# ruanhuabin/DataCompressionFloat

Hardware: AMD Instinct MI355X
Metric: compress + decompress GB/s (input floats), bit-exact round trip (higher is better)
Workload: dtype u8

## Files before the change

datacompressionfloat_amd/_lib.py:

```python
import ctypes
import os

_HERE = os.path.dirname(os.path.abspath(__file__))
LIB_PATH = os.environ.get("MRCZ_LIB_PATH") or os.path.join(_HERE, "lib", "libmrcz_hip.so")


class MrczLibraryMissing(ImportError):
    pass


class MrczBoxGeom(ctypes.Structure):
    _fields_ = [("data_word0", ctypes.c_uint64), ("nx", ctypes.c_uint32), ("ny", ctypes.c_uint32), ("nz", ctypes.c_uint32),
                ("bx", ctypes.c_uint32), ("by", ctypes.c_uint32), ("bz", ctypes.c_uint32), ("fill_bits", ctypes.c_uint32)]


class MrczBinGeom(ctypes.Structure):
    _fields_ = [("data_word0", ctypes.c_uint64), ("nx", ctypes.c_uint32), ("ny", ctypes.c_uint32), ("nz", ctypes.c_uint32),
                ("fx", ctypes.c_uint32), ("fy", ctypes.c_uint32), ("fz", ctypes.c_uint32)]


class MrczCompare(ctypes.Structure):
    _fields_ = [(k, ctypes.c_uint64) for k in ("n", "n_header_diff", "n_diff", "n_finite", "n_special_diff", "n_over_abs", "n_over_rel",
                                               "first_over", "max_err_index", "max_rel_index")] + \
               [(k, ctypes.c_double) for k in ("max_err", "max_rel", "sum_err", "sum_abs_err", "sum_err2", "orig_min", "orig_max",
# ... 39 lines not shown
    lib.mrcz_record_size.restype = i32
    lib.mrcz_record_size.argtypes = [vp, u32, ctypes.POINTER(u64)]
    lib.mrcz_records_index.restype = i32
    lib.mrcz_records_index.argtypes = [vp, u64, u64, u32, ctypes.POINTER(u64)]
    lib.mrcz_uncompress_range.restype = i32
    lib.mrcz_uncompress_range.argtypes = [vp, vp, u64, u64, u32, u64, u64, u64, vp, i32, ctypes.POINTER(u64)]
    geom = ctypes.POINTER(MrczBoxGeom)
    lib.mrcz_box_origins.restype = i32
    lib.mrcz_box_origins.argtypes = [geom, vp, u32, vp]
    lib.mrcz_boxes_chunks.restype = i32
    lib.mrcz_boxes_chunks.argtypes = [geom, vp, u32, u64, u32, vp]
    lib.mrcz_uncompress_boxes.restype = i32
    lib.mrcz_uncompress_boxes.argtypes = [vp, vp, u64, u64, u32, u64, u64, geom, vp, u32, vp, i32, ctypes.POINTER(u64)]
    bgeom = ctypes.POINTER(MrczBinGeom)
    lib.mrcz_bin_chunks.restype = i32
    lib.mrcz_bin_chunks.argtypes = [bgeom, u64, u32, ctypes.POINTER(u64), ctypes.POINTER(u64)]
    lib.mrcz_uncompress_binned.restype = i32
    lib.mrcz_uncompress_binned.argtypes = [vp, vp, u64, u64, u32, u64, u64, bgeom, vp, i32, ctypes.POINTER(u64)]
    lib.mrcz_binned_finish.restype = i32
    lib.mrcz_binned_finish.argtypes = [vp, bgeom, vp, vp]
    lib.mrcz_uncompress_compare.restype = i32
    lib.mrcz_uncompress_compare.argtypes = [vp, vp, u64, u64, u32, u64, u64, vp, ctypes.c_double, ctypes.c_double, i32, vp]
    lib.mrcz_compare_finish.restype = i32
    lib.mrcz_compare_finish.argtypes = [vp, vp, u64, u64, ctypes.POINTER(MrczCompare)]
    lib.mrcz_crc32_combine.restype = u32
    lib.mrcz_crc32_combine.argtypes = [u32, u32, u64]
    lib.mrcz_uncompress_digest.restype = i32
    lib.mrcz_uncompress_digest.argtypes = [vp, vp, u64, u64, u32, u64, u64, i32, vp]
    for f in (lib.mrcz_digest_words, lib.mrcz_digest_words_async):
        f.restype = i32
        f.argtypes = [vp, vp, u64, u64, u32, i32, i32, ctypes.c_float, vp]
    lib.mrcz_digest_finish.restype = i32
    lib.mrcz_digest_finish.argtypes = [vp, vp, u64, u64, ctypes.POINTER(MrczDigest)]
    lib.mrcz_record_top_span.restype = i32
    lib.mrcz_record_top_span.argtypes = [vp, u32, i32, ctypes.POINTER(u64), ctypes.POINTER(u64)]
    lib.mrcz_uncompress_top.restype = i32
    lib.mrcz_uncompress_top.argtypes = [vp, vp, u64, u64, u32, u64, u64, i32, i32, vp, ctypes.POINTER(u64)]
    lib.mrcz_generate_kat_words.restype = i32
    lib.mrcz_generate_kat_words.argtypes = [vp, vp, u64, u64]
    lib.mrcz_set_ztypes.restype = i32
    lib.mrcz_set_ztypes.argtypes = [vp, ctypes.c_char_p]
    lib.mrcz_erase_bits.restype = i32
    lib.mrcz_erase_bits.argtypes = [vp, vp, u64, u64, i32]
    lib.mrcz_erase_abs.restype = i32
    lib.mrcz_erase_abs.argtypes = [vp, vp, u64, u64, ctypes.c_float]
    lib.mrcz_set_timing.restype = i32
    lib.mrcz_set_timing.argtypes = [vp, i32]
    lib.mrcz_last_timings.restype = i32
    lib.mrcz_last_timings.argtypes = [vp, ctypes.POINTER(ctypes.c_char_p), ctypes.POINTER(ctypes.c_float), i32]
    lib.mrcz_debug_fallbacks.restype = ctypes.c_int64
    lib.mrcz_debug_fallbacks.argtypes = [vp]
    lib.mrcz_debug_chain_fallbacks.restype = ctypes.c_int64
    lib.mrcz_debug_chain_fallbacks.argtypes = [vp]
    return lib


EXPORTS = [
    "mrcz_create", "mrcz_destroy", "mrcz_last_error", "mrcz_stream", "mrcz_records_bound",
    "mrcz_compress_chunks", "mrcz_uncompress_chunks", "mrcz_erase_bits", "mrcz_set_timing",
    "mrcz_last_timings", "mrcz_debug_blocks", "mrcz_debug_fallbacks", "mrcz_debug_chain_fallbacks", "mrcz_debug_inflate_phases", "mrcz_debug_candidates", "mrcz_device_count", "mrcz_dev_malloc", "mrcz_dev_free",
    "mrcz_host_malloc", "mrcz_host_free", "mrcz_copy_h2d", "mrcz_copy_d2h",
    "mrcz_event_create", "mrcz_event_destroy", "mrcz_event_record", "mrcz_stream_wait_event", "mrcz_event_sync",
    "mrcz_copy_h2d_async", "mrcz_copy_d2h_async", "mrcz_compress_chunks_async", "mrcz_uncompress_chunks_async",
    "mrcz_set_ztypes", "mrcz_generate_kat_words", "mrcz_err_hist", "mrcz_err_collect", "mrcz_compress_chunks_int8", "mrcz_uncompress_chunks_int8", "mrcz_compress_chunks_int8_async", "mrcz_uncompress_chunks_int8_async",
    "mrcz_record_size", "mrcz_records_index", "mrcz_uncompress_range", "mrcz_uncompress_range_async",
    "mrcz_box_origins", "mrcz_boxes_chunks", "mrcz_uncompress_boxes",
    "mrcz_bin_chunks", "mrcz_uncompress_binned", "mrcz_binned_finish",
    "mrcz_compress_chunks_abs", "mrcz_compress_chunks_abs_async", "mrcz_erase_abs",
    "mrcz_uncompress_compare", "mrcz_compare_finish",
    "mrcz_crc32_combine", "mrcz_uncompress_digest", "mrcz_digest_words", "mrcz_digest_words_async", "mrcz_digest_finish",
    "mrcz_record_top_span", "mrcz_uncompress_top", "mrcz_uncompress_top_async",
]
```

datacompressionfloat_amd/csrc/mrcz_api.hip:

```cpp
#include "mrcz_compress.hip"
#include "mrcz_huffman.hip"
#include "mrcz_inflate.hip"
#include "mrcz_inflate_par.hip"
#include "mrcz_tools.hip"

#include "../../include/mrcz_hip.h"

#include <math.h>
#include <stdio.h>
#include <stdlib.h>
#include <string.h>
#include <time.h>

using namespace mrcz;

#define MAX_TIMERS 32

constexpr int MAX_LANES = 2;
constexpr uint32_t SPLIT_PCT = 55;
constexpr uint32_t HIST_FEW = 8;
constexpr uint32_t BLK_WGS_PER_CU = 3;
static uint32_t validate_grid(uint32_t ns) { return ns * 192u < 4096u ? 4096u : ns * 192u > 32768u ? 32768u : ns * 192u; }

namespace mrcz { struct CmpPart; }
// ... 278 lines not shown
    if (!(eps > 0.0f) || !isfinite(eps)) return fail(ctx, MRCZ_EINVAL, "absolute error bound must be finite and > 0", hipSuccess);
    uint32_t bits;
    memcpy(&bits, &eps, 4);
    const int32_t e = (int32_t)(bits >> 23);
    ae->q = e ? e - 127 : -150 + (32 - __builtin_clz(bits));
    ae->E = bits;
    return MRCZ_OK;
}

static int ensure_planes(mrcz_ctx *ctx)
{
    if (ctx->planes) return MRCZ_OK;
    hipError_t e = hipMalloc((void **)&ctx->planes, (size_t)4 * ctx->row_chunks * CHK);
    if (e != hipSuccess) { ctx->planes = NULL; return fail(ctx, MRCZ_ENOMEM, "plane workspace", e); }
    return MRCZ_OK;
}

static int compress_lane(mrcz_ctx *ctx, hipStream_t lstream, int phase, int slot, uint32_t s0, const uint32_t *bin, uint64_t bfl,
                         uint32_t nb, uint32_t mask, uint32_t fstart, uint8_t *out, Xform xf, AbsErr ae)
{
    const uint32_t ns = 4u * nb;
    TileSum *tsum = ctx->tsum + (size_t)s0 * TPS;
    TileInfo *tinfo = ctx->tinfo + (size_t)s0 * TPS;
    StreamInfo *sinfo = ctx->sinfo + s0;
    uint32_t *blkstart = ctx->blkstart + (size_t)s0 * (MAXBLK + 1);
    uint32_t *slideq = ctx->slideq + (size_t)s0 * MAXSLIDE;
    uint16_t *pairhist = ctx->pairhist + (size_t)s0 * MAXPAIR * HROW;
    uint16_t *blkfreq = ctx->blkfreq + (size_t)s0 * MAXBLK * HROW;
    uint32_t *blkcode = ctx->blkcode + (size_t)s0 * MAXBLK * HROW;
    uint32_t *blkhdr = ctx->blkhdr + (size_t)s0 * MAXBLK * HDRWORDS;
    BlkMeta *meta = ctx->meta + (size_t)s0 * MAXBLK;
    BlkLay *lay = ctx->lay + (size_t)s0 * MAXBLK;
    uint32_t *pairbits = ctx->pairbits + (size_t)s0 * MAXPAIR;
    uint32_t *pairoff = ctx->pairoff + (size_t)s0 * MAXPAIR;
    uint32_t *blkbase = ctx->blkbase + s0 + (uint32_t)slot;
    uint8_t *planes = ctx->planes + (size_t)s0 * CHK;
    if (phase == 0) {
        if (xf == Xform::Quant) LAUNCH("k_tile_summary", k_tile_summary<Xform::Quant>, dim3(SPS, nb), dim3(256), bin, bfl, mask, fstart, tsum, planes);
        else if (xf == Xform::AbsErr) LAUNCH("k_tile_summary", k_tile_summary<Xform::AbsErr>, dim3(SPS, nb), dim3(256), bin, bfl, ae, fstart, tsum, planes);
        else LAUNCH("k_tile_summary", k_tile_summary<Xform::Mask>, dim3(SPS, nb), dim3(256), bin, bfl, mask, fstart, tsum, planes);
        LAUNCH("k_stream_scan", k_stream_scan, dim3(ns), dim3(256), tsum, bfl, tinfo, sinfo, blkstart);
        if (nb <= 12u) LAUNCH("k_histogram", k_histogram<4>, dim3(SPS, nb, 4), dim3(256), planes, bfl, tinfo, pairhist, blkstart, slideq, HIST_FEW);
        else LAUNCH("k_histogram", k_histogram<1>, dim3(SPS, nb, 4), dim3(64), planes, bfl, tinfo, pairhist, blkstart, slideq, HIST_FEW);
        LAUNCH("k_block_reduce", k_block_reduce, dim3(MAXBLK, ns), dim3(64), tinfo, sinfo, pairhist, blkfreq);
        LAUNCH("k_block_index", k_block_index, dim3(1), dim3(256), sinfo, ns, blkbase);
        HIPCHK(hipEventRecord(ctx->ev_stream[slot], lstream), "event");
        unsigned long long *hdbg = ctx->phase_profile == 3 ? ctx->dbgphase : (unsigned long long *)NULL;
        LAUNCH("k_huffman", k_huffman, dim3((ns * MAXBLK + HUFF_TREES - 1) / HUFF_TREES), dim3(HUFF_TREES), sinfo, ns, blkbase, blkfreq, blkcode, blkhdr, meta, hdbg);
        LAUNCH("k_huffman_hdr", k_huffman_hdr, dim3(ns * MAXBLK), dim3(64), sinfo, ns, blkbase, blkcode, blkhdr, meta);
        LAUNCH("k_stream_layout", k_stream_layout, dim3(ns), dim3(64), sinfo, meta, blkstart, slideq, lay);
        LAUNCH("k_pair_bits", k_pair_bits, dim3(SPS, ns), dim3(64), sinfo, lay, pairhist, blkcode, tinfo, pairbits);
        LAUNCH("k_pair_offsets", k_pair_offsets, dim3(ns), dim3(64), sinfo, lay, tinfo, pairbits, pairoff);
    } else if (phase == 1) {
        LAUNCH("k_container", k_container, dim3(1), dim3(256), sinfo, nb, out, ctx->result, 0, slot);
    } else {
        LAUNCH("k_zero_records", k_zero_records, dim3(2048), dim3(256), out, ctx->result, slot);
        LAUNCH("k_container", k_container, dim3(1), dim3(256), sinfo, nb, out, ctx->result, 1, slot);
        LAUNCH("k_emit", k_emit, dim3(SPS, nb, 4), dim3(64), planes, bfl, tinfo, sinfo, lay, blkstart, blkcode, pairoff, out);
        LAUNCH("k_emit_headers", k_emit_headers, dim3(MAXBLK + 1, ns), dim3(64), sinfo, lay, meta, blkhdr, blkstart, out);
    }
    return MRCZ_OK;
}

static int compress_enqueue(mrcz_ctx_t *ctx, const void *d_in, uint64_t nfloats, uint64_t first_chunk, int bits, void *d_out, uint64_t out_cap,
                            uint64_t *h_res, Xform xf, AbsErr ae = AbsErr{})
{
    if (!ctx || !d_in || !d_out || !h_res) return MRCZ_EINVAL;
    if (bits < 0 || bits > 32) return fail(ctx, MRCZ_EINVAL, "bits outside 0..32 (reference table has 33 entries, workers.c:29-37)", hipSuccess);
    if (((uintptr_t)d_in & 15u) || ((uintptr_t)d_out & 3u)) return fail(ctx, MRCZ_EINVAL, "d_in must be 16-byte and d_out 4-byte aligned", hipSuccess);
    ctx->ntimers = 0;
    if (nfloats == 0) return fail(ctx, MRCZ_EINVAL, "nothing to compress", hipSuccess);
    const uint64_t bound = mrcz_records_bound(nfloats);
    if (out_cap < bound) return fail(ctx, MRCZ_ECAP, "output capacity below mrcz_records_bound()", hipSuccess);
    HIPCHK(hipSetDevice(ctx->device), "hipSetDevice");
    const uint32_t mask = mask_of(bits);
    const uint64_t nchunks = (nfloats + CHK - 1) / CHK;
    const uint32_t *in = (const uint32_t *)d_in;
    uint8_t *out = (uint8_t *)d_out;
    if (int rc = ensure_planes(ctx)) return rc;
    HIPCHK(hipMemsetAsync(ctx->result, 0, 16 * sizeof(uint64_t), ctx->stream), "memset result");
    HIPCHK(hipEventRecord(ctx->ev_start, ctx->stream), "event");
    for (uint32_t l = 1; l < ctx->lanes; l++) HIPCHK(hipStreamWaitEvent(ctx->lane_stream[l], ctx->ev_start, 0), "wait");
    bool cont_pending = false;
    uint32_t prev_lanes = 0, prev_lc0[MAX_LANES + 1] = {0};
    int stream_pending = -1;
    for (uint64_t c0 = 0; c0 < nchunks; c0 += ctx->max_chunks) {
        const uint32_t nb = (uint32_t)((nchunks - c0) < ctx->max_chunks ? (nchunks - c0) : ctx->max_chunks);
        const uint32_t nlanes = (ctx->timing || nb < 8u) ? 1u : ctx->lanes;
        const uint64_t bfl = (nfloats - c0 * CHK) < (uint64_t)nb * CHK ? (nfloats - c0 * CHK) : (uint64_t)nb * CHK;
        ctx->last_streams = 4u * nb;
        ctx->last_nlanes = nlanes;
        uint32_t lc0[MAX_LANES + 1] = {0u, nb};
        if (nlanes == 2u) {
            lc0[1] = (uint32_t)(((uint64_t)nb * SPLIT_PCT + 50u) / 100u);
            if (lc0[1] < 1u) lc0[1] = 1u;
            if (lc0[1] > nb - 1u) lc0[1] = nb - 1u;
            lc0[2] = nb;
        }
        bool same_rows = prev_lanes == nlanes;
        for (uint32_t l = 0; same_rows && l < nlanes; l++) same_rows = prev_lc0[l] == lc0[l];
        if (prev_lanes && !same_rows) {
            for (uint32_t l = 0; l < prev_lanes; l++) HIPCHK(hipEventRecord(ctx->ev_done[l], ctx->lane_stream[l]), "event");
            for (uint32_t l = 0; l < nlanes; l++)
                for (uint32_t k = 0; k < prev_lanes; k++)
                    if (k != l) HIPCHK(hipStreamWaitEvent(ctx->lane_stream[l], ctx->ev_done[k], 0), "wait");
        }
        prev_lanes = nlanes;
        for (uint32_t l = 0; l <= nlanes; l++) prev_lc0[l] = lc0[l];
        for (int phase = 0; phase < 3; phase++) {
            for (uint32_t l = 0; l < nlanes; l++) {
                const uint32_t cb = lc0[l], nbl = lc0[l + 1] - lc0[l];
// ... 502 lines not shown
    return MRCZ_OK;
}

extern "C" int mrcz_err_collect(mrcz_ctx_t *ctx, const void *d_orig, const void *d_dec, uint64_t n, uint64_t base_index, uint32_t threshold_bits,
                                void *d_points, uint64_t cap_points, uint64_t count_in, uint64_t *count_out)
{
    if (!ctx || !d_orig || !d_dec || !d_points || !count_out) return MRCZ_EINVAL;
    HIPCHK(hipSetDevice(ctx->device), "hipSetDevice");
    ctx->ntimers = 0;
    hipStream_t lstream = ctx->stream;
    if (!ctx->errhist) {
        hipError_t e = hipMalloc((void **)&ctx->errhist, 2049 * sizeof(unsigned long long));
        if (e != hipSuccess) { ctx->errhist = NULL; return fail(ctx, MRCZ_ENOMEM, "error histogram", e); }
    }
    unsigned long long *cnt = ctx->errhist + 2048;
    unsigned long long start = count_in;
    HIPCHK(hipMemcpyAsync(cnt, &start, sizeof(start), hipMemcpyHostToDevice, ctx->stream), "copy count");
    if (n) LAUNCH("k_err_collect", k_err_collect, dim3(2048), dim3(256), (const uint32_t *)d_orig, (const uint32_t *)d_dec, n, base_index, threshold_bits,
                  (ErrPoint *)d_points, cnt, cap_points);
    unsigned long long got = 0;
    HIPCHK(hipMemcpyAsync(&got, cnt, sizeof(got), hipMemcpyDeviceToHost, ctx->stream), "copy count");
    HIPCHK(hipStreamSynchronize(ctx->stream), "stream sync (collect)");
    *count_out = got;
    return MRCZ_OK;
}

extern "C" int mrcz_debug_inflate_phases(mrcz_ctx_t *ctx, int enable, uint32_t stream, uint64_t out[20])
{
    if (!ctx) return MRCZ_EINVAL;
    ctx->phase_profile = enable;
    if (enable == 3 && !out && hipMemset(ctx->dbgphase, 0, 40 * sizeof(unsigned long long)) != hipSuccess) return MRCZ_EHIP;
    if (out) {
        if (stream >= 8u * ctx->max_chunks) return MRCZ_EINVAL;
        if (hipMemcpy(out, ctx->dbgphase + (size_t)stream * 20, 20 * sizeof(uint64_t), hipMemcpyDeviceToHost) != hipSuccess) return MRCZ_EHIP;
    }
    return MRCZ_OK;
}

extern "C" int mrcz_debug_candidates(mrcz_ctx_t *ctx, uint64_t out[2])
{
    if (!ctx || !out) return MRCZ_EINVAL;
    uint32_t raw[RAW_SEGS];
    if (hipMemcpy(raw, ctx->njobs + 4, sizeof(raw), hipMemcpyDeviceToHost) != hipSuccess) return MRCZ_EHIP;
    out[0] = 0;
    for (uint32_t g = 0; g < RAW_SEGS; g++) out[0] += raw[g];
    out[1] = 0;
    uint32_t nc[512];
    const uint32_t ns = 4u * (ctx->max_chunks < 128u ? ctx->max_chunks : 128u);
    if (hipMemcpy(nc, ctx->ncand, ns * sizeof(uint32_t), hipMemcpyDeviceToHost) != hipSuccess) return MRCZ_EHIP;
    for (uint32_t s = 0; s < ns; s++) out[1] += nc[s];
    return MRCZ_OK;
}

extern "C" int64_t mrcz_debug_fallbacks(const mrcz_ctx_t *ctx) { return ctx ? (int64_t)ctx->last_fallbacks : -1; }
extern "C" int64_t mrcz_debug_chain_fallbacks(mrcz_ctx_t *ctx) { return ctx ? (int64_t)ctx->last_chain_fallbacks : -1; }

extern "C" int mrcz_debug_blocks(mrcz_ctx_t *ctx, uint32_t stream, mrcz_block_info_t *blocks, uint32_t max_blocks)
{
    if (!ctx || stream >= ctx->last_streams) return MRCZ_EINVAL;
    {
        uint32_t l = 0;
        while (l + 1 < ctx->last_nlanes && (stream >> 2) >= ctx->last_lc0[l + 1]) l++;
        stream = ctx->last_row0[l] + (stream - 4u * ctx->last_lc0[l]);
    }
    StreamInfo si;
    if (hipMemcpy(&si, ctx->sinfo + stream, sizeof(si), hipMemcpyDeviceToHost) != hipSuccess) return MRCZ_EHIP;
    uint32_t nb = si.nblk;
    if (nb > (uint32_t)MAXBLK) return MRCZ_EFORMAT;
    BlkLay *lay = (BlkLay *)malloc(sizeof(BlkLay) * (nb + 1));
    BlkMeta *meta = (BlkMeta *)malloc(sizeof(BlkMeta) * (nb + 1));
    uint32_t *bs = (uint32_t *)malloc(sizeof(uint32_t) * (nb + 2));
    (void)hipMemcpy(lay, ctx->lay + (size_t)stream * MAXBLK, sizeof(BlkLay) * nb, hipMemcpyDeviceToHost);
    (void)hipMemcpy(meta, ctx->meta + (size_t)stream * MAXBLK, sizeof(BlkMeta) * nb, hipMemcpyDeviceToHost);
    (void)hipMemcpy(bs, ctx->blkstart + (size_t)stream * (MAXBLK + 1), sizeof(uint32_t) * (nb + 1), hipMemcpyDeviceToHost);
    for (uint32_t b = 0; b < nb && b < max_blocks; b++) {
        blocks[b].start = bs[b];
        blocks[b].end = bs[b + 1];
        blocks[b].btype = lay[b].btype;
        blocks[b].opt_len = meta[b].opt_len;
        blocks[b].static_len = meta[b].static_len;
        blocks[b].bitpos = lay[b].bitpos;
    }
    free(lay); free(meta); free(bs);
    return (int)nb;
}
```

datacompressionfloat_amd/csrc/mrcz_compress.hip:

```cpp
#include "mrcz_tile.h"

namespace mrcz {

template <Xform X>
__global__ __launch_bounds__(256) void k_tile_summary(const uint32_t *__restrict__ in, uint64_t nfloats,
                                                      typename XformArg<X>::type mask, uint32_t first_chunk_is_file_start,
                                                      TileSum *__restrict__ tsum, uint8_t *__restrict__ planes)
{
    __shared__ __attribute__((aligned(16))) uint8_t lds[4 * PLANE_LDS];
    const uint32_t g = blockIdx.x, c = blockIdx.y;
    const uint64_t cbase = (uint64_t)c * CHK;
    const uint32_t n = (uint32_t)((nfloats - cbase) < CHK ? (nfloats - cbase) : CHK);
    if ((uint64_t)g * SEG >= n) return;
    const uint32_t *cin = in + cbase;
    const uint32_t unmasked = (c == 0 && first_chunk_is_file_start) ? 256u : 0u;
    const int lane = lane_id(), w = threadIdx.x >> 6;
    const uint32_t s = 4u * c + (uint32_t)w;

    for (int ti = 0; ti < TILES_PER_SEG; ti++) {
        const uint32_t t0 = g * SEG + ti * TILE;
        if (t0 >= n) break;
        const int len = (int)((n - t0) < (uint32_t)TILE ? (n - t0) : (uint32_t)TILE);
        stage_tile<X>(cin, t0, (uint32_t)len, mask, unmasked, lds);
        __syncthreads();
// ... 566 lines not shown
    }
}

__global__ __launch_bounds__(64) void k_pair_offsets(const StreamInfo *__restrict__ sinfo, const BlkLay *__restrict__ lay,
                                                     const TileInfo *__restrict__ tinfo, const uint32_t *__restrict__ pairbits,
                                                     uint32_t *__restrict__ pairoff)
{
    __shared__ uint32_t s_val[MAXPAIR];
    __shared__ uint8_t s_head[MAXPAIR];
    const uint32_t s = blockIdx.x;
    const StreamInfo si = sinfo[s];
    const int lane = lane_id();
    const TileInfo *ti = tinfo + (size_t)s * TPS;
    const uint32_t npair = si.nseg ? si.nseg + si.nsym / BLK_SYMS : 0u;
    for (uint32_t g = lane; g < si.nseg; g += 64) {
        const uint32_t bs = ti[g * TILES_PER_SEG].P / BLK_SYMS;
        const uint32_t be = ((g + 1 < si.nseg) ? ti[(g + 1) * TILES_PER_SEG].P : si.nsym) / BLK_SYMS;
        for (uint32_t b = bs; b <= be; b++) {
            const uint32_t i = g + b;
            if (i >= (uint32_t)MAXPAIR) break;
            const bool head = b > bs || g == 0u;
            s_head[i] = head ? 1 : 0;
            s_val[i] = head ? (b < si.nblk ? lay[(size_t)s * MAXBLK + b].databit : 0u) : pairbits[(size_t)s * MAXPAIR + i - 1u];
        }
    }
    __builtin_amdgcn_wave_barrier();
    constexpr int R = (MAXPAIR + 63) / 64;
    const uint32_t per = (npair + 63u) / 64u;
    const uint32_t i0 = (uint32_t)lane * per;
    uint32_t sum = 0, flag = 0;
#pragma unroll
    for (int r = 0; r < R; r++) {
        const uint32_t i = i0 + (uint32_t)r;
        if ((uint32_t)r >= per || i >= npair) continue;
        if (s_head[i]) { sum = s_val[i]; flag = 1; } else sum += s_val[i];
    }
    uint32_t isum = sum, iflag = flag;
    for (int d = 1; d < 64; d <<= 1) {
        const uint32_t os = (uint32_t)__shfl_up((int)isum, d), of = (uint32_t)__shfl_up((int)iflag, d);
        if (lane >= d) { if (!iflag) isum += os; iflag |= of; }
    }
    uint32_t run = (uint32_t)__shfl_up((int)isum, 1);
    if (lane == 0) run = 0;
    uint32_t *po = pairoff + (size_t)s * MAXPAIR;
#pragma unroll
    for (int r = 0; r < R; r++) {
        const uint32_t i = i0 + (uint32_t)r;
        if ((uint32_t)r >= per || i >= npair) continue;
        run = s_head[i] ? s_val[i] : run + s_val[i];
        po[i] = run;
    }
}

__global__ __launch_bounds__(256) void k_zero_records(uint8_t *__restrict__ out, const uint64_t *__restrict__ result, int slot)
{
    uint8_t *b = out + result[8 + slot], *e = out + result[12 + slot];
    uint8_t *ba = reinterpret_cast<uint8_t *>(((uintptr_t)b + 15u) & ~(uintptr_t)15u);
    uint8_t *ea = reinterpret_cast<uint8_t *>((uintptr_t)e & ~(uintptr_t)15u);
    if (ba > e) ba = e;
    if (ea < ba) ea = ba;
    if (blockIdx.x == 0 && threadIdx.x < 16u && b + threadIdx.x < ba) b[threadIdx.x] = 0;
    if (blockIdx.x == 1 && threadIdx.x < 16u && ea + threadIdx.x < e) ea[threadIdx.x] = 0;
    uint4 *p = reinterpret_cast<uint4 *>(ba);
    const uint64_t n = (uint64_t)(ea - ba) >> 4;
    const uint4 z = make_uint4(0, 0, 0, 0);
    for (uint64_t i = (uint64_t)blockIdx.x * 256u + threadIdx.x; i < n; i += (uint64_t)gridDim.x * 256u) p[i] = z;
}

__global__ __launch_bounds__(256) void k_container(StreamInfo *__restrict__ sinfo, uint32_t nchunks, uint8_t *__restrict__ out,
                                                   uint64_t *__restrict__ result ,
                                                   int write_headers, int slot)
{
    __shared__ SegPair wsum[4];
    const uint32_t c = threadIdx.x;
    uint32_t len[4] = {0, 0, 0, 0}, raw[4] = {0, 0, 0, 0};
    SegPair v;
    v.sum = 0;
    v.brk = 0;
    if (c < nchunks) {
        for (int j = 0; j < 4; j++) {
            len[j] = sinfo[4 * c + j].paylen;
            raw[j] = sinfo[4 * c + j].raw;
        }
        v.sum = 16u + len[0] + len[1] + len[2] + len[3];
    }
    const uint64_t base = write_headers ? result[8 + slot] : result[0];
    const SegPair pre = block_excl_scan(v, wsum);
    if (c < nchunks) {
        const uint64_t off = base + pre.sum;
        uint64_t p = off + 16;
        for (int j = 0; j < 4; j++) {
            if (write_headers) {
                uint8_t *h = out + off + 4u * j;
                h[0] = (uint8_t)(len[j] & 0xff);
                h[1] = (uint8_t)((len[j] >> 8) & 0xff);
                h[2] = (uint8_t)((len[j] >> 16) & 0xff);
                h[3] = (uint8_t)(((len[j] >> 24) & 0x7f) | (raw[j] << 7));
            } else {
                sinfo[4 * c + j].payoff = p;
                atomicAdd((unsigned long long *)&result[1 + j], (unsigned long long)len[j] + 4ull);
            }
            p += len[j];
        }
    }
    __syncthreads();
    if (!write_headers && c + 1 == nchunks) {
        result[8 + slot] = base;
        result[12 + slot] = base + pre.sum + v.sum;
        result[0] = base + pre.sum + v.sum;
    }
}

constexpr int STAGE_WORDS = 1280;

__device__ __forceinline__ void global_or_bits(uint32_t *out32, uint64_t pos, uint32_t val, int nbits)
{
    if (nbits <= 0) return;
    const uint64_t wi = pos >> 5;
    const int sh = (int)(pos & 31u);
    const uint64_t v = (uint64_t)(nbits >= 32 ? val : (val & ((1u << nbits) - 1u))) << sh;
    if ((uint32_t)v) atomicOr(&out32[wi], (uint32_t)v);
    if ((uint32_t)(v >> 32)) atomicOr(&out32[wi + 1], (uint32_t)(v >> 32));
}

struct LanePacker {
    uint32_t *stage;
    uint64_t acc;
    int nacc;
    uint32_t word;
    int covered;
};
__device__ __forceinline__ void packer_init(LanePacker &p, uint32_t *stage, uint32_t bitpos)
{
    p.stage = stage;
    p.word = bitpos >> 5;
    p.covered = (int)(bitpos & 31u);
    p.acc = 0;
    p.nacc = 0;
}
__device__ __forceinline__ void packer_put(LanePacker &p, uint32_t val, int nbits)
{
    p.acc |= (uint64_t)val << (p.covered + p.nacc);
    p.nacc += nbits;
    if (p.covered + p.nacc >= 32) {
        const uint32_t wv = (uint32_t)p.acc;
        if (p.covered == 0) p.stage[p.word] = wv;
        else atomicOr(&p.stage[p.word], wv);
        p.acc >>= 32;
        p.nacc -= 32 - p.covered;
        p.covered = 0;
        p.word++;
    }
}
__device__ __forceinline__ void packer_finish(LanePacker &p)
{
    if (p.nacc > 0) atomicOr(&p.stage[p.word], (uint32_t)p.acc);
}

constexpr int EMIT_WAVES = 5;
#define OPAQUE4(x, q) asm volatile("" : "+v"((x)[4 * (q)]), "+v"((x)[4 * (q) + 1]), "+v"((x)[4 * (q) + 2]), "+v"((x)[4 * (q) + 3]))

__device__ __forceinline__ uint32_t quarter_byte(const uint32_t wv[4], int j)
// ... 8 lines not shown
    if (__ballot(Lg != 0xffffu) == 0ull) {
#pragma unroll
        for (int j = 0; j < 16; j++) bits += lut[(wv[j >> 2] >> (8 * (j & 3))) & 0xffu] >> 16;
    } else {
#pragma unroll
        for (int j = 0; j < 16; j++) {
            const uint32_t e = lut[(wv[j >> 2] >> (8 * (j & 3))) & 0xffu];
            bits += ((Lg >> j) & 1u) ? (e >> 16) : 0u;
        }
    }
    return bits;
}

__device__ __forceinline__ void quarter_emit(LanePacker &pk, const uint32_t *lut, const uint32_t wv[4], uint32_t Sg, uint32_t Mg,
                                             int q, const LaneTile &lt, uint32_t dbits)
{
    if (__ballot(Mg != 0u || Sg != 0xffffu) == 0ull) {
#pragma unroll
        for (int j = 0; j < 16; j += 2) {
            const uint32_t e0 = lut[(wv[j >> 2] >> (8 * (j & 3))) & 0xffu];
            const uint32_t e1 = lut[(wv[(j + 1) >> 2] >> (8 * ((j + 1) & 3))) & 0xffu];
            const uint32_t n0 = e0 >> 16;
            packer_put(pk, (e0 & 0xffffu) | ((e1 & 0xffffu) << n0), (int)(n0 + (e1 >> 16)));
        }
        return;
    }
    uint32_t rem = Sg;
    while (__ballot(rem != 0u)) {
        if (rem) {
            const int j = __builtin_ctz(rem);
            rem &= rem - 1u;
            uint32_t val;
            int nb;
            if ((Mg >> j) & 1u) {
                int xb, xv;
                const int code = len_code(match_len_at(lt.E, lt.a, lt.nextS, 16 * q + j), &xb, &xv);
                const uint32_t e = lut[257 + code];
                const int cl = (int)(e >> 16);
                val = (e & 0xffffu) | ((uint32_t)xv << cl);
                nb = cl + xb + (int)dbits;
            } else {
                const uint32_t e = lut[quarter_byte(wv, j)];
                val = e & 0xffffu;
                nb = (int)(e >> 16);
            }
            packer_put(pk, val, nb);
        }
    }
}

__global__ __launch_bounds__(64) __attribute__((amdgpu_waves_per_eu(EMIT_WAVES))) void k_emit(const uint8_t *__restrict__ planes, uint64_t nfloats, const TileInfo *__restrict__ tinfo,
                                              const StreamInfo *__restrict__ sinfo, const BlkLay *__restrict__ lay,
                                              const uint32_t *__restrict__ blkstart, const uint32_t *__restrict__ blkcode,
                                              const uint32_t *__restrict__ pairoff, uint8_t *__restrict__ out)
{
    __shared__ __attribute__((aligned(16))) uint32_t stage[STAGE_WORDS];
    __shared__ uint32_t lut[HROW];
    const uint32_t g = blockIdx.x, c = blockIdx.y;
    const uint64_t cbase = (uint64_t)c * CHK;
    const uint32_t n = (uint32_t)((nfloats - cbase) < CHK ? (nfloats - cbase) : CHK);
    if ((uint64_t)g * SEG >= n) return;
    const int lane = lane_id(), w = plane_of_slot(blockIdx.z);
    const uint32_t s = 4u * c + (uint32_t)w;
    const uint8_t *pl = planes + (size_t)s * CHK;
    const StreamInfo si = sinfo[s];
    uint32_t *out32 = reinterpret_cast<uint32_t *>(out);
    const uint64_t paybit = si.payoff * 8ull;
    const uint32_t *bstart = blkstart + (size_t)s * (MAXBLK + 1);
    const BlkLay *blay = lay + (size_t)s * MAXBLK;

    uint32_t curBlk = 0xffffffffu;
    uint32_t cur = 0;
    int mode = -1;
    uint32_t blkEnd = 0;
    uint32_t dbits = 0;

    for (int ti = 0; ti < TILES_PER_SEG; ti++) {
        const uint32_t t0 = g * SEG + ti * TILE;
        if (t0 >= n) break;
        const int len = (int)((n - t0) < (uint32_t)TILE ? (n - t0) : (uint32_t)TILE);
        uint32_t x[16];
        load_plane_row(pl, t0, len, lane, x);
        if (si.raw) {
            uint8_t *dst = out + si.payoff + t0 + 64u * (uint32_t)lane;
            const int mine = len - 64 * lane;
            if (mine >= 64) {
#pragma unroll
                for (int k = 0; k < 4; k++) {
                    const uint4 v = make_uint4(x[4 * k], x[4 * k + 1], x[4 * k + 2], x[4 * k + 3]);
                    __builtin_memcpy(dst + 16 * k, &v, 16);
                }
            } else {
                for (int i = 0; i < mine; i++) dst[i] = pl[t0 + 64u * (uint32_t)lane + (uint32_t)i];
            }
            continue;
        }
        const TileInfo tinf = tinfo[(size_t)s * TPS + (t0 / TILE)];
        const LaneTile lt = analyse_lane(x, lane, len, tinf.B, tinf.F);
        const LaneCls cls = classify_lane(lt.E, lt.a, lt.prevS, lt.nextS);
        if (curBlk == 0xffffffffu) {
            curBlk = tinf.P / BLK_SYMS;
            if (bstart[curBlk] > t0) curBlk--;
            mode = -1;
        }

        int pos0 = 0;
        int cap = len;
        for (int part = 0; part < 16 && pos0 < len; part++) {
            if (mode < 0 || t0 + (uint32_t)pos0 >= blkEnd) {
                if (mode >= 0) curBlk++;
                const BlkLay L = blay[curBlk];
                mode = (int)L.btype;
                blkEnd = bstart[curBlk + 1];
                if (mode == 0) cur = L.databit + 8u * (t0 + (uint32_t)pos0 - bstart[curBlk]);
                else {
                    __builtin_amdgcn_wave_barrier();
                    if (mode == 2) {
                        const uint32_t *code = blkcode + ((size_t)s * MAXBLK + curBlk) * HROW;
                        for (int i = lane; i < 286; i += 64) lut[i] = code[i];
                        dbits = 1;
                    } else {
                        for (int i = lane; i < 286; i += 64) {
                            int l;
                            const uint32_t cd = static_lcode(i, &l);
                            lut[i] = cd | ((uint32_t)l << 16);
                        }
                        dbits = 5;
                    }
                    cur = pairoff[(size_t)s * MAXPAIR + (g + curBlk)];
                    __builtin_amdgcn_wave_barrier();
                }
            }
            int pos1 = cap;
            if (blkEnd < t0 + (uint32_t)pos1) pos1 = (int)(blkEnd - t0);

            if (mode == 0) {
                const uint32_t nbytes = (uint32_t)(pos1 - pos0);
                const uint64_t dg = si.payoff + (cur >> 3);
                const uint32_t mis = (uint32_t)(dg & 3u);
                const uint64_t w0 = dg >> 2;
                const uint32_t nwords = (mis + nbytes + 3u) >> 2;
                const uint8_t *src = pl + t0 + (uint32_t)pos0;
                for (uint32_t k = lane; k < nwords; k += 64) {
                    uint32_t v = 0;
                    bool full = true;
#pragma unroll
                    for (int j = 0; j < 4; j++) {
                        const int rel = (int)(4u * k + (uint32_t)j) - (int)mis;
                        if (rel >= 0 && rel < (int)nbytes) v |= (uint32_t)src[rel] << (8 * j);
                        else full = false;
                    }
                    if (full) out32[w0 + k] = v;
                    else if (v) atomicOr(&out32[w0 + k], v);
                }
                cur += 8u * nbytes;
                pos0 = pos1; cap = len;
                continue;
            }
            const int lo = pos0 - lt.a, hi = pos1 - lt.a;
            const uint64_t mlo = lo <= 0 ? ~0ull : (lo >= 64 ? 0ull : (~0ull << lo));
            const uint64_t mhi = hi >= 64 ? ~0ull : (hi <= 0 ? 0ull : ((1ull << hi) - 1ull));
            const uint64_t pm = mlo & mhi & lt.V;
            const uint64_t S = cls.S & pm, M = cls.M & pm;

            if (__ballot(S != 0ull) == 0ull) { pos0 = pos1; cap = len; continue; }
            uint32_t lbits = 0;
            {
                const uint64_t L = S & ~M;
#pragma unroll
                for (int q = 0; q < 4; q++) {
                    const uint32_t Lg = (uint32_t)(L >> (16 * q)) & 0xffffu;
                    if (__ballot(Lg != 0u) == 0ull) continue;
                    OPAQUE4(x, q);
                    lbits += quarter_literal_bits(lut, &x[4 * q], Lg);
                }
                uint64_t m = M;
                while (m) {
                    const int i = ctz64(m); m &= m - 1;
                    int xb, xv;
                    const int code = len_code(match_len_at(lt.E, lt.a, lt.nextS, i), &xb, &xv);
                    lbits += (lut[257 + code] >> 16) + (uint32_t)xb + dbits;
                }
            }
            uint32_t tot;
            const uint32_t lofs = wave_excl_sum(lbits, &tot);
            if (tot) {
                const uint64_t gbit = paybit + cur;
                const uint32_t lead = (uint32_t)(gbit & 31u);
                const uint32_t nwords = (lead + tot + 31u) >> 5;
                if (nwords > (uint32_t)STAGE_WORDS) {
                    cap = pos0 + ((((pos1 - pos0) >> 1) + 63) & ~63);
                    continue;
                }
                for (uint32_t i = lane; i < nwords; i += 64) stage[i] = 0;
                __builtin_amdgcn_wave_barrier();
                LanePacker pk;
                packer_init(pk, stage, lead + lofs);
#pragma unroll
                for (int q = 0; q < 4; q++) {
                    const uint32_t Sg = (uint32_t)(S >> (16 * q)) & 0xffffu, Mg = (uint32_t)(M >> (16 * q)) & 0xffffu;
                    if (__ballot(Sg != 0u) == 0ull) continue;
                    OPAQUE4(x, q);
                    quarter_emit(pk, lut, &x[4 * q], Sg, Mg, q, lt, dbits);
                }
                packer_finish(pk);
                __builtin_amdgcn_wave_barrier();
                const uint64_t w0 = gbit >> 5;
                for (uint32_t i = lane; i < nwords; i += 64) {
                    const uint32_t v = stage[i];
                    if (i == 0 || i == nwords - 1) { if (v) atomicOr(&out32[w0 + i], v); }
                    else out32[w0 + i] = v;
                }
                __builtin_amdgcn_wave_barrier();
                cur += tot;
            }
            pos0 = pos1; cap = len;
        }
    }
}

__global__ __launch_bounds__(64) void k_emit_headers(const StreamInfo *__restrict__ sinfo, const BlkLay *__restrict__ lay,
                                                     const BlkMeta *__restrict__ meta, const uint32_t *__restrict__ blkhdr,
                                                     const uint32_t *__restrict__ blkstart, uint8_t *__restrict__ out)
{
    const uint32_t b = blockIdx.x, s = blockIdx.y;
    const StreamInfo si = sinfo[s];
    if (si.raw || b > si.nblk) return;
    const int lane = lane_id();
    uint32_t *out32 = reinterpret_cast<uint32_t *>(out);
    const uint64_t paybit = si.payoff * 8ull;
    if (b == si.nblk) {
        if (lane == 0) {
            const uint32_t mb = ((si.zbits + 3u + 7u) & ~7u) + 16u;
            global_or_bits(out32, paybit + mb, 0xffffu, 16);
        }
        return;
    }
    const BlkLay L = lay[(size_t)s * MAXBLK + b];
    const BlkMeta m = meta[(size_t)s * MAXBLK + b];
    if (L.btype == 0) {
        if (lane == 0) {
            const uint32_t slen = blkstart[(size_t)s * (MAXBLK + 1) + b + 1] - blkstart[(size_t)s * (MAXBLK + 1) + b];
            global_or_bits(out32, paybit + L.databit - 32u, (slen & 0xffffu) | ((~slen & 0xffffu) << 16), 32);
        }
        return;
    }
    if (L.btype == 1) {
        if (lane == 0) {
            global_or_bits(out32, paybit + L.bitpos, 2u, 3);
            int l;
            const uint32_t cd = static_lcode(256, &l);
            global_or_bits(out32, paybit + L.endbit - (uint32_t)l, cd, l);
        }
        return;
    }
    if (lane == 0) {
        global_or_bits(out32, paybit + L.bitpos, 4u, 3);
        global_or_bits(out32, paybit + L.endbit - (m.eob >> 16), m.eob & 0xffffu, (int)(m.eob >> 16));
    }
    const uint32_t *h = blkhdr + ((size_t)s * MAXBLK + b) * HDRWORDS;
    const uint32_t nw = (m.hdr_bits + 31u) >> 5;
    for (uint32_t i = lane; i < nw; i += 64) {
        const uint32_t nb = (i + 1 == nw) ? (m.hdr_bits - 32u * i) : 32u;
        global_or_bits(out32, paybit + L.bitpos + 3u + 32u * i, h[i], (int)nb);
    }
}

}
```

include/mrcz_hip.h:

```cpp
#ifndef MRCZ_HIP_H_
#define MRCZ_HIP_H_

#include <stddef.h>
#include <stdint.h>

#ifdef __cplusplus
extern "C" {
#endif

#define MRCZ_CHUNK_FLOATS 6291456u
#define MRCZ_FILE_HEADER_BYTES 17

#define MRCZ_OK 0
#define MRCZ_EINVAL (-1)
#define MRCZ_ENOMEM (-2)
#define MRCZ_ECAP (-3)
#define MRCZ_EFORMAT (-4)
#define MRCZ_EHIP (-5)

typedef struct mrcz_ctx mrcz_ctx_t;

int mrcz_create(mrcz_ctx_t **ctx, int device, uint32_t max_batch_chunks);
void mrcz_destroy(mrcz_ctx_t *ctx);
const char *mrcz_last_error(const mrcz_ctx_t *ctx);
// ... 103 lines not shown

#define MRCZ_DIGEST_NONE 0
#define MRCZ_DIGEST_MASK 1
#define MRCZ_DIGEST_INT8 2
#define MRCZ_DIGEST_ABS 3
typedef struct mrcz_digest {
    uint32_t crc32;
    uint32_t reserved;
    uint64_t nbytes;
} mrcz_digest_t;
uint32_t mrcz_crc32_combine(uint32_t crc_a, uint32_t crc_b, uint64_t nbytes_b);
int mrcz_uncompress_digest(mrcz_ctx_t *ctx, const void *d_records, uint64_t len, uint64_t nfloats_file, uint32_t chk,
                           uint64_t first_chunk, uint64_t nchunks, int int_mode, mrcz_digest_t *d_acc);
int mrcz_digest_words(mrcz_ctx_t *ctx, const void *d_words, uint64_t nwords, uint64_t first_chunk, uint32_t chk, int xform,
                      int bits, float eps, mrcz_digest_t *d_acc);
int mrcz_digest_words_async(mrcz_ctx_t *ctx, const void *d_words, uint64_t nwords, uint64_t first_chunk, uint32_t chk, int xform,
                            int bits, float eps, mrcz_digest_t *d_acc);
int mrcz_digest_finish(mrcz_ctx_t *ctx, const mrcz_digest_t *d_acc, uint64_t first_chunk, uint64_t nchunks,
                       mrcz_digest_t *h_total);

#define MRCZ_TOP_F32 0
#define MRCZ_TOP_U16 1
#define MRCZ_TOP_THINNED 4
int mrcz_record_top_span(const void *h_header16, uint32_t n, int keep, uint64_t *skip, uint64_t *bytes);
int mrcz_uncompress_top(mrcz_ctx_t *ctx, const void *d_records, uint64_t len, uint64_t nfloats_file, uint32_t chk,
                        uint64_t first_chunk, uint64_t nchunks, int keep, int flags, void *d_out, uint64_t *consumed);
int mrcz_uncompress_top_async(mrcz_ctx_t *ctx, const void *d_records, uint64_t len, uint64_t nfloats_file, uint32_t chk,
                              uint64_t first_chunk, uint64_t nchunks, int keep, int flags, void *d_out, uint64_t *h_result3);

int mrcz_erase_bits(mrcz_ctx_t *ctx, void *d_words, uint64_t nwords, uint64_t first_word_index, int bits);

int mrcz_err_hist(mrcz_ctx_t *ctx, const void *d_orig, const void *d_dec, uint64_t n, int pass, uint32_t prefix, int reset,
                  uint64_t hist[2048]);
int mrcz_err_collect(mrcz_ctx_t *ctx, const void *d_orig, const void *d_dec, uint64_t n, uint64_t base_index, uint32_t threshold_bits,
                     void *d_points, uint64_t cap_points, uint64_t count_in, uint64_t *count_out);

int mrcz_generate_kat_words(mrcz_ctx_t *ctx, void *d_words, uint64_t first_index, uint64_t nwords);

int mrcz_set_timing(mrcz_ctx_t *ctx, int on);

int mrcz_last_timings(const mrcz_ctx_t *ctx, const char **names, float *ms, int max);

typedef struct {
    uint32_t start, end;
    uint32_t btype;
    uint32_t opt_len, static_len;
    uint32_t bitpos;
} mrcz_block_info_t;
int mrcz_debug_blocks(mrcz_ctx_t *ctx, uint32_t stream, mrcz_block_info_t *blocks, uint32_t max_blocks);

int64_t mrcz_debug_fallbacks(const mrcz_ctx_t *ctx);
int64_t mrcz_debug_chain_fallbacks(mrcz_ctx_t *ctx);

int mrcz_debug_inflate_phases(mrcz_ctx_t *ctx, int enable, uint32_t stream, uint64_t out[20]);

int mrcz_debug_candidates(mrcz_ctx_t *ctx, uint64_t out[2]);

#ifdef __cplusplus
}
#endif
#endif
```

Baseline: 218.2.

## Replace full record zeroing with targeted boundary clearing and carried partial words in emit

Drops the kernel that zeroed the whole output record region and the second header-writing container launch. A new kernel clears only the bit ranges that emit ORs into: pair boundaries, block headers and EOB tails. k_emit now carries a partial trailing word between consecutive emits, so most stage words become plain stores instead of atomicOr. Stored-block edges are written bytewise. Any missed bit range would leave stale output and break the bit-exact round trip, and the change adds an atomic debug counter for emit splits.

New measurement: 225.1, median of 6. 3.1% higher.

```diff
diff --git a/datacompressionfloat_amd/_lib.py b/datacompressionfloat_amd/_lib.py
--- a/datacompressionfloat_amd/_lib.py
+++ b/datacompressionfloat_amd/_lib.py
@@ -115,13 +115,15 @@
     lib.mrcz_debug_fallbacks.argtypes = [vp]
     lib.mrcz_debug_chain_fallbacks.restype = ctypes.c_int64
     lib.mrcz_debug_chain_fallbacks.argtypes = [vp]
+    lib.mrcz_debug_emit_splits.restype = ctypes.c_int64
+    lib.mrcz_debug_emit_splits.argtypes = [vp]
     return lib
 
 
 EXPORTS = [
     "mrcz_create", "mrcz_destroy", "mrcz_last_error", "mrcz_stream", "mrcz_records_bound",
     "mrcz_compress_chunks", "mrcz_uncompress_chunks", "mrcz_erase_bits", "mrcz_set_timing",
-    "mrcz_last_timings", "mrcz_debug_blocks", "mrcz_debug_fallbacks", "mrcz_debug_chain_fallbacks", "mrcz_debug_inflate_phases", "mrcz_debug_candidates", "mrcz_device_count", "mrcz_dev_malloc", "mrcz_dev_free",
+    "mrcz_last_timings", "mrcz_debug_blocks", "mrcz_debug_fallbacks", "mrcz_debug_chain_fallbacks", "mrcz_debug_emit_splits", "mrcz_debug_inflate_phases", "mrcz_debug_candidates", "mrcz_device_count", "mrcz_dev_malloc", "mrcz_dev_free",
     "mrcz_host_malloc", "mrcz_host_free", "mrcz_copy_h2d", "mrcz_copy_d2h",
     "mrcz_event_create", "mrcz_event_destroy", "mrcz_event_record", "mrcz_stream_wait_event", "mrcz_event_sync",
     "mrcz_copy_h2d_async", "mrcz_copy_d2h_async", "mrcz_compress_chunks_async", "mrcz_uncompress_chunks_async",
diff --git a/datacompressionfloat_amd/csrc/mrcz_api.hip b/datacompressionfloat_amd/csrc/mrcz_api.hip
--- a/datacompressionfloat_amd/csrc/mrcz_api.hip
+++ b/datacompressionfloat_amd/csrc/mrcz_api.hip
@@ -354,11 +354,10 @@
         LAUNCH("k_pair_bits", k_pair_bits, dim3(SPS, ns), dim3(64), sinfo, lay, pairhist, blkcode, tinfo, pairbits);
         LAUNCH("k_pair_offsets", k_pair_offsets, dim3(ns), dim3(64), sinfo, lay, tinfo, pairbits, pairoff);
     } else if (phase == 1) {
-        LAUNCH("k_container", k_container, dim3(1), dim3(256), sinfo, nb, out, ctx->result, 0, slot);
+        LAUNCH("k_container", k_container, dim3(1), dim3(256), sinfo, nb, out, ctx->result);
     } else {
-        LAUNCH("k_zero_records", k_zero_records, dim3(2048), dim3(256), out, ctx->result, slot);
-        LAUNCH("k_container", k_container, dim3(1), dim3(256), sinfo, nb, out, ctx->result, 1, slot);
-        LAUNCH("k_emit", k_emit, dim3(SPS, nb, 4), dim3(64), planes, bfl, tinfo, sinfo, lay, blkstart, blkcode, pairoff, out);
+        LAUNCH("k_clear_boundaries", k_clear_boundaries, dim3(MAXBLK + 1, ns), dim3(64), sinfo, lay, meta, pairoff, out);
+        LAUNCH("k_emit", k_emit, dim3(SPS, nb, 4), dim3(64), planes, bfl, tinfo, sinfo, lay, blkstart, blkcode, pairoff, out, ctx->result);
         LAUNCH("k_emit_headers", k_emit_headers, dim3(MAXBLK + 1, ns), dim3(64), sinfo, lay, meta, blkhdr, blkstart, out);
     }
     return MRCZ_OK;
@@ -967,6 +966,14 @@
     return MRCZ_OK;
 }
 
+extern "C" int64_t mrcz_debug_emit_splits(mrcz_ctx_t *ctx)
+{
+    if (!ctx) return -1;
+    uint64_t v = 0;
+    if (hipSetDevice(ctx->device) != hipSuccess || hipMemcpy(&v, ctx->result + 8, sizeof(v), hipMemcpyDeviceToHost) != hipSuccess) return -1;
+    return (int64_t)v;
+}
+
 extern "C" int64_t mrcz_debug_fallbacks(const mrcz_ctx_t *ctx) { return ctx ? (int64_t)ctx->last_fallbacks : -1; }
 extern "C" int64_t mrcz_debug_chain_fallbacks(mrcz_ctx_t *ctx) { return ctx ? (int64_t)ctx->last_chain_fallbacks : -1; }
 
diff --git a/datacompressionfloat_amd/csrc/mrcz_compress.hip b/datacompressionfloat_amd/csrc/mrcz_compress.hip
--- a/datacompressionfloat_amd/csrc/mrcz_compress.hip
+++ b/datacompressionfloat_amd/csrc/mrcz_compress.hip
@@ -642,24 +642,8 @@
     }
 }
 
-__global__ __launch_bounds__(256) void k_zero_records(uint8_t *__restrict__ out, const uint64_t *__restrict__ result, int slot)
-{
-    uint8_t *b = out + result[8 + slot], *e = out + result[12 + slot];
-    uint8_t *ba = reinterpret_cast<uint8_t *>(((uintptr_t)b + 15u) & ~(uintptr_t)15u);
-    uint8_t *ea = reinterpret_cast<uint8_t *>((uintptr_t)e & ~(uintptr_t)15u);
-    if (ba > e) ba = e;
-    if (ea < ba) ea = ba;
-    if (blockIdx.x == 0 && threadIdx.x < 16u && b + threadIdx.x < ba) b[threadIdx.x] = 0;
-    if (blockIdx.x == 1 && threadIdx.x < 16u && ea + threadIdx.x < e) ea[threadIdx.x] = 0;
-    uint4 *p = reinterpret_cast<uint4 *>(ba);
-    const uint64_t n = (uint64_t)(ea - ba) >> 4;
-    const uint4 z = make_uint4(0, 0, 0, 0);
-    for (uint64_t i = (uint64_t)blockIdx.x * 256u + threadIdx.x; i < n; i += (uint64_t)gridDim.x * 256u) p[i] = z;
-}
-
 __global__ __launch_bounds__(256) void k_container(StreamInfo *__restrict__ sinfo, uint32_t nchunks, uint8_t *__restrict__ out,
-                                                   uint64_t *__restrict__ result ,
-                                                   int write_headers, int slot)
+                                                   uint64_t *__restrict__ result )
 {
     __shared__ SegPair wsum[4];
     const uint32_t c = threadIdx.x;
@@ -674,30 +658,66 @@
         }
         v.sum = 16u + len[0] + len[1] + len[2] + len[3];
     }
-    const uint64_t base = write_headers ? result[8 + slot] : result[0];
+    const uint64_t base = result[0];
     const SegPair pre = block_excl_scan(v, wsum);
     if (c < nchunks) {
         const uint64_t off = base + pre.sum;
         uint64_t p = off + 16;
         for (int j = 0; j < 4; j++) {
-            if (write_headers) {
-                uint8_t *h = out + off + 4u * j;
-                h[0] = (uint8_t)(len[j] & 0xff);
-                h[1] = (uint8_t)((len[j] >> 8) & 0xff);
-                h[2] = (uint8_t)((len[j] >> 16) & 0xff);
-                h[3] = (uint8_t)(((len[j] >> 24) & 0x7f) | (raw[j] << 7));
-            } else {
-                sinfo[4 * c + j].payoff = p;
-                atomicAdd((unsigned long long *)&result[1 + j], (unsigned long long)len[j] + 4ull);
-            }
+            uint8_t *h = out + off + 4u * j;
+            h[0] = (uint8_t)(len[j] & 0xff);
+            h[1] = (uint8_t)((len[j] >> 8) & 0xff);
+            h[2] = (uint8_t)((len[j] >> 16) & 0xff);
+            h[3] = (uint8_t)(((len[j] >> 24) & 0x7f) | (raw[j] << 7));
+            sinfo[4 * c + j].payoff = p;
+            atomicAdd((unsigned long long *)&result[1 + j], (unsigned long long)len[j] + 4ull);
             p += len[j];
         }
     }
     __syncthreads();
-    if (!write_headers && c + 1 == nchunks) {
-        result[8 + slot] = base;
-        result[12 + slot] = base + pre.sum + v.sum;
-        result[0] = base + pre.sum + v.sum;
+    if (c + 1 == nchunks) result[0] = base + pre.sum + v.sum;
+}
+
+__device__ __forceinline__ void clear_payload_bits(uint8_t *out, uint64_t pb, uint64_t pe , uint32_t lo,
+                                                   uint32_t hi , int lane)
+{
+    if (hi <= lo) return;
+    const uint64_t w0 = (pb * 8ull + lo) >> 5, w1 = (pb * 8ull + hi - 1u) >> 5;
+    for (uint64_t w = w0 + (uint64_t)lane; w <= w1; w += 64u) {
+        const uint64_t b = 4ull * w;
+        if (b >= pb && b + 4u <= pe) reinterpret_cast<uint32_t *>(out)[w] = 0u;
+        else
+            for (uint64_t j = b; j < b + 4u; j++)
+                if (j >= pb && j < pe) out[j] = 0;
+    }
+}
+
+__global__ __launch_bounds__(64) void k_clear_boundaries(const StreamInfo *__restrict__ sinfo, const BlkLay *__restrict__ lay,
+                                                         const BlkMeta *__restrict__ meta, const uint32_t *__restrict__ pairoff,
+                                                         uint8_t *__restrict__ out)
+{
+    const uint32_t b = blockIdx.x, s = blockIdx.y;
+    const StreamInfo si = sinfo[s];
+    if (si.raw) return;
+    const int lane = lane_id();
+    const uint64_t pb = si.payoff, pe = si.payoff + si.paylen;
+    const uint32_t npair = si.nseg ? si.nseg + si.nsym / BLK_SYMS : 0u;
+    for (uint32_t i = b * 64u + (uint32_t)lane; i < npair; i += gridDim.x * 64u) {
+        const uint32_t p = pairoff[(size_t)s * MAXPAIR + i];
+        clear_payload_bits(out, pb, pe, p ? p - 1u : 0u, p + 1u, 0);
+    }
+    if (b > si.nblk) return;
+    if (b == si.nblk) {
+        clear_payload_bits(out, pb, pe, si.zbits, 8u * si.paylen, lane);
+        return;
+    }
+    const BlkLay L = lay[(size_t)s * MAXBLK + b];
+    clear_payload_bits(out, pb, pe, L.bitpos, L.databit, lane);
+    if (L.btype != 0u) {
+        int l = 0;
+        if (L.btype == 1u) (void)static_lcode(256, &l);
+        else l = (int)(meta[(size_t)s * MAXBLK + b].eob >> 16);
+        clear_payload_bits(out, pb, pe, L.endbit - (uint32_t)l, L.endbit, lane);
     }
 }
 
@@ -812,7 +832,8 @@
 __global__ __launch_bounds__(64) __attribute__((amdgpu_waves_per_eu(EMIT_WAVES))) void k_emit(const uint8_t *__restrict__ planes, uint64_t nfloats, const TileInfo *__restrict__ tinfo,
                                               const StreamInfo *__restrict__ sinfo, const BlkLay *__restrict__ lay,
                                               const uint32_t *__restrict__ blkstart, const uint32_t *__restrict__ blkcode,
-                                              const uint32_t *__restrict__ pairoff, uint8_t *__restrict__ out)
+                                              const uint32_t *__restrict__ pairoff, uint8_t *__restrict__ out,
+                                              uint64_t *__restrict__ result )
 {
     __shared__ __attribute__((aligned(16))) uint32_t stage[STAGE_WORDS];
     __shared__ uint32_t lut[HROW];
@@ -834,6 +855,9 @@
     int mode = -1;
     uint32_t blkEnd = 0;
     uint32_t dbits = 0;
+    uint32_t carry = 0;
+    bool have_carry = false;
+    bool carry_shared = false;
 
     for (int ti = 0; ti < TILES_PER_SEG; ti++) {
         const uint32_t t0 = g * SEG + ti * TILE;
@@ -868,6 +892,10 @@
         int cap = len;
         for (int part = 0; part < 16 && pos0 < len; part++) {
             if (mode < 0 || t0 + (uint32_t)pos0 >= blkEnd) {
+                if (have_carry) {
+                    if (lane == 0 && carry) atomicOr(&out32[(paybit + cur) >> 5], carry);
+                    have_carry = false;
+                }
                 if (mode >= 0) curBlk++;
                 const BlkLay L = blay[curBlk];
                 mode = (int)L.btype;
@@ -911,7 +939,13 @@
                         else full = false;
                     }
                     if (full) out32[w0 + k] = v;
-                    else if (v) atomicOr(&out32[w0 + k], v);
+                    else {
+#pragma unroll
+                        for (int j = 0; j < 4; j++) {
+                            const int rel = (int)(4u * k + (uint32_t)j) - (int)mis;
+                            if (rel >= 0 && rel < (int)nbytes) out[4u * (w0 + k) + (uint32_t)j] = (uint8_t)(v >> (8 * j));
+                        }
+                    }
                 }
                 cur += 8u * nbytes;
                 pos0 = pos1; cap = len;
@@ -950,9 +984,12 @@
                 const uint32_t nwords = (lead + tot + 31u) >> 5;
                 if (nwords > (uint32_t)STAGE_WORDS) {
                     cap = pos0 + ((((pos1 - pos0) >> 1) + 63) & ~63);
+                    if (lane == 0) atomicAdd((unsigned long long *)&result[8], 1ull);
                     continue;
                 }
+                const bool first_shared = lead != 0u && (!have_carry || carry_shared);
                 for (uint32_t i = lane; i < nwords; i += 64) stage[i] = 0;
+                if (have_carry && lane == 0) stage[0] = carry;
                 __builtin_amdgcn_wave_barrier();
                 LanePacker pk;
                 packer_init(pk, stage, lead + lofs);
@@ -966,17 +1003,25 @@
                 packer_finish(pk);
                 __builtin_amdgcn_wave_barrier();
                 const uint64_t w0 = gbit >> 5;
-                for (uint32_t i = lane; i < nwords; i += 64) {
+                const bool open_end = ((lead + tot) & 31u) != 0u;
+                const uint32_t nout = open_end ? nwords - 1u : nwords;
+                for (uint32_t i = lane; i < nout; i += 64) {
                     const uint32_t v = stage[i];
-                    if (i == 0 || i == nwords - 1) { if (v) atomicOr(&out32[w0 + i], v); }
+                    if (i == 0 && first_shared) { if (v) atomicOr(&out32[w0], v); }
                     else out32[w0 + i] = v;
                 }
+                if (open_end) {
+                    carry = (uint32_t)__builtin_amdgcn_readfirstlane((int)stage[nwords - 1u]);
+                    carry_shared = nwords == 1u && first_shared;
+                }
+                have_carry = open_end;
                 __builtin_amdgcn_wave_barrier();
                 cur += tot;
             }
             pos0 = pos1; cap = len;
         }
     }
+    if (have_carry && lane == 0 && carry) atomicOr(&out32[(paybit + cur) >> 5], carry);
 }
 
 __global__ __launch_bounds__(64) void k_emit_headers(const StreamInfo *__restrict__ sinfo, const BlkLay *__restrict__ lay,
diff --git a/include/mrcz_hip.h b/include/mrcz_hip.h
--- a/include/mrcz_hip.h
+++ b/include/mrcz_hip.h
@@ -179,6 +179,8 @@
 int64_t mrcz_debug_fallbacks(const mrcz_ctx_t *ctx);
 int64_t mrcz_debug_chain_fallbacks(mrcz_ctx_t *ctx);
 
+int64_t mrcz_debug_emit_splits(mrcz_ctx_t *ctx);
+
 int mrcz_debug_inflate_phases(mrcz_ctx_t *ctx, int enable, uint32_t stream, uint64_t out[20]);
 
 int mrcz_debug_candidates(mrcz_ctx_t *ctx, uint64_t out[2]);
```
